# nunofonseca/fastq_utils

Hardware: AMD Instinct MI355X
Metric: Mreads/s validated (fastq_info, 150bp) (higher is better)
Workload: dtype u8

## Files before the change

### fastq_utils_amd/csrc/fqg_abi.hip

```cpp
#include <hip/hip_runtime.h>

#include <cstring>
#include <rocprim/rocprim.hpp>

#include <algorithm>
#include <cmath>
#include <memory>
#include <mutex>
#include <optional>
#include <cstdio>
#include <cstdlib>
#include <cstring>
#include <string>
#include <vector>

#include "fqg_device.h"
#include "fqg_kernels.hip"
#include "fqg_stream_kernels.hip"
#include "fqg_index_kernels.hip"
#include "fqg_names_build_kernels.hip"
#include "fqg_barcode_kernels.hip"
#include "fqg_census_kernels.hip"
#include "fqg_filter_kernels.hip"
#include "fqg_umi_kernels.hip"
// ... 710 lines not shown
  RecordDuties rd;
  int want_names;
  bool want_index;
  StreamOut so{};
  NameCapture nc{};
  ChunkRanks cr{};
  uint32_t n_parts = 1;
  int last_pct = 16;
  uint64_t early_line_cap = 0;
  uint64_t todo_steps_cap = 0;
  LinesArgs PA{};
  uint64_t n_newlines = 0, n_lines_all = 0, line_cap = 0, limit = 0;
  bool index_lost = false;

  uint32_t boot_span() const { return (uint32_t)std::min<uint64_t>(kStreamBootBytes, nbytes & ~255ull); }
  uint32_t part_begin(uint32_t part) const {
    if (part == 0 || n_parts <= 1) return part == 0 ? 0u : n_spans;
    if (part >= n_parts) return n_spans;
    const uint32_t last = std::min<uint32_t>(n_spans - (n_parts - 1), std::max<uint32_t>(1u, (uint32_t)((uint64_t)n_spans * (uint32_t)last_pct / 100u)));
    return (uint32_t)((uint64_t)(n_spans - last) * part / (n_parts - 1));
  }
  LinesArgs lines_args(const fqg_ctx* c, const ChunkRanks& cr, AccState* acc, unsigned long long* hist, const IndexMode& ix) const {
    LinesArgs A{};
    A.img = img;
    A.n = nbytes;
    A.cr = cr;
    A.stage = (const uint16_t*)c->stage.p;
    A.line_end = ix.line_end;
    A.line_cap = ix.line_cap;
    A.suspect_bits = sm.bits;
    A.suspect_cap = sm.cap;
    A.flags = sm.flags;
    A.space = rd.space;
    A.weight = rd.weight;
    A.acc = acc;
    A.hist = hist;
    A.no_index = ix.no_index ? 1u : 0u;
    A.index_only = 0u;
    A.keep_from = ix.keep_from;
    return A;
  }
};

ChunkRanks chunk_ranks(const fqg_ctx* c, uint32_t n_chunks) {
  ChunkRanks cr;
  cr.counts = (const uint32_t*)c->tile_counts.p;
  cr.local = (const uint32_t*)c->tile_local.p;
  cr.span_excl = (const unsigned long long*)c->span_sums.p;
  cr.n_chunks = n_chunks;
  return cr;
}

void fold_parted(fqg_ctx* c, AccState* dst, unsigned long long* dst_hist) {
  hipLaunchKernelGGL(k_acc_merge, dim3(64), dim3(kBlock), 0, c->stream, c->pipe_acc, c->pipe_hist, dst, dst_hist, dst ? 0 : 1);
  hipLaunchKernelGGL(k_acc_scratch_reset, dim3(1), dim3(1), 0, c->stream, c->pipe_acc);
  c->pipe_dirty = false;
}

int resident_per_cu(int& asked, const void* kernel) {
  if (!asked) {
    int nb = 0;
    if (hipOccupancyMaxActiveBlocksPerMultiprocessor(&nb, kernel, kBlock, 0) != hipSuccess || nb < 1) nb = 4;
    asked = nb;
  }
  return asked;
}

int stream_begin(fqg_ctx* c, StreamCall& s) {
  int rc;
  if ((rc = ensure(c, c->tile_counts, (size_t)s.n_chunks * 4))) return rc;
  if ((rc = ensure(c, c->tile_local, (size_t)s.n_chunks * 4))) return rc;
  if ((rc = ensure(c, c->span_sums, (size_t)s.n_spans * 8))) return rc;
  if ((rc = ensure(c, c->cinfo, (size_t)s.n_chunks * 4))) return rc;
  if ((rc = ensure(c, c->redo, (size_t)s.n_chunks * 4))) return rc;
  if ((rc = ensure(c, c->stage, (size_t)s.n_chunks * kStageCap * 2))) return rc;
  if ((rc = ensure(c, c->queue, (size_t)kStreamQueueCap * 8))) return rc;
  init_call_state(c);
  HIP_TRY(c, hipMemcpyAsync(c->d_cs, c->h_cs, sizeof(CallState), hipMemcpyHostToDevice, c->stream));
  s.so.counts = (uint32_t*)c->tile_counts.p;
  s.so.cinfo = (uint32_t*)c->cinfo.p;
  s.so.stage = (uint16_t*)c->stage.p;
  s.so.queue = (unsigned long long*)c->queue.p;
  s.so.queue_cap = kStreamQueueCap;
  s.cr = chunk_ranks(c, s.n_chunks);
  ProfScope ps(c, "k_stream_boot");
  hipLaunchKernelGGL(k_stream_boot, dim3(1), dim3(kBootBlock), 0, c->stream, s.img, s.boot_span(), c->d_cs);
  return 0;
}

int stream_name_setup(fqg_ctx* c, StreamCall& s) {
  int rc;
  if ((rc = read_call_state(c))) return rc;
  const double per_chunk = (double)(c->h_cs->boot_lines / 4 + 1) * (double)kChunkBytes / (double)std::max<uint32_t>(s.boot_span(), 1);
  uint32_t shift = 3;
  while (shift < 7 && (double)(1u << shift) < 1.25 * per_chunk + 1.0) ++shift;
  s.nc.K = 1u << shift;
  s.nc.fmt = s.rd.fmt;
  s.nc.is_pe = s.rd.is_pe;
  if ((rc = ensure(c, c->name_recs, ((size_t)s.n_chunks << shift) * (s.want_names == 2 ? kDigestWords : kNameRecWords) * 8))) return rc;
  if ((rc = ensure(c, c->name_hcount, (size_t)s.n_chunks * 2))) return rc;
  s.nc.recs = (unsigned long long*)c->name_recs.p;
  s.nc.hcount = (uint16_t*)c->name_hcount.p;
  c->names.k_shift = shift;
  return 0;
}

int stream_plan_parts(fqg_ctx* c, StreamCall& s) {
  int rc;
// ... 1764 lines not shown
```

### fastq_utils_amd/csrc/fqg_device.h

```cpp
#pragma once
#include <hip/hip_runtime.h>
#include <stdint.h>

#include "../../include/fqg.h"

namespace fqg {

constexpr int kWave = 64;
constexpr int kBlock = 256;
constexpr int kChunkBytes = 4096;
constexpr int kSlices = kChunkBytes / (kWave * 16);
constexpr int kScanSpan = 4096;
constexpr uint64_t kNoRecord = ~0ull;

constexpr uint32_t kFlagNul = 1u;
constexpr uint32_t kFlagCr = 2u;
constexpr uint32_t kFlagHigh = 8u;
constexpr uint32_t kFlagSuspectOverflow = 16u;
constexpr uint32_t kFlagStageOverflow = 32u;
constexpr uint32_t kFlagQueueOverflow = 64u;

constexpr int kStageCap = 256;
constexpr uint32_t kClsAt = 1u, kClsPlus = 2u;
constexpr uint32_t kInfoUnknown = 4u, kInfoRange = 8u, kInfoOneLine = 16u, kInfoNotBases = 32u;
// ... 2 lines not shown
  return (info & kInfoUnknown) || (info & 3u) != (rank0 & 3u);
}
__host__ __device__ inline bool chunk_info_range(uint32_t info, uint32_t rank0) {
  if (!(info & kInfoRange)) return false;
  return (info & kInfoOneLine) ? (rank0 & 3u) == 3u : true;
}

constexpr uint32_t kNameRecWords = 8;
constexpr uint32_t kNameRecText = 60;
constexpr uint32_t kNameInline = 56;
constexpr uint32_t kNoCapture = 0xFFFFu;
struct NameCapture {
  unsigned long long* recs;
  uint16_t* hcount;
  uint32_t K;
  int fmt, is_pe;
};
constexpr uint32_t kDigestWords = 2;
constexpr uint32_t kDigestText = 64;
constexpr uint32_t kDigestAt = 1u << 29, kDigestOk = 1u << 30;

__host__ __device__ constexpr uint64_t name_mul(uint32_t k) {
  return (0x9E3779B97F4A7C15ull + (uint64_t)k * 0xD1B54A32D192ED03ull) | 1ull;
}
__host__ __device__ constexpr uint32_t name_key_a(uint32_t k) { return (uint32_t)name_mul(k); }
__host__ __device__ constexpr uint32_t name_key_b(uint32_t k) { return (uint32_t)(name_mul(k) >> 32); }
__device__ __forceinline__ uint64_t name_word(uint64_t sum, uint64_t w, uint32_t k) {
  return sum + (uint64_t)((uint32_t)w + name_key_a(k)) * (uint64_t)((uint32_t)(w >> 32) + name_key_b(k));
}
__device__ __forceinline__ uint64_t name_seed(uint32_t n) { return 0x2545F4914F6CDD1Dull + (uint64_t)n; }
__device__ __forceinline__ uint64_t name_fin(uint64_t h) {
  const uint32_t hi = (uint32_t)(h >> 32), t = (uint32_t)h ^ hi;
  const uint64_t p = (uint64_t)t * 0xD6E8FEB9u, q = (uint64_t)hi * 0x85EBCA6Bu;
  return p ^ ((q << 32) | (q >> 32));
}

struct CallState {
  unsigned long long first_key;
  unsigned long long stop_record;
  unsigned long long n_newlines;
  unsigned long long aux0, aux1;
  unsigned long long list_count;
  unsigned int flags;
  unsigned int last_byte_is_nl;
  unsigned int qmin_byte, qmax_byte;
  unsigned long long queue_count;
  unsigned int redo_count;
  unsigned int boot_qmin, boot_qmax;
  unsigned int boot_lines;
  unsigned int pad_;
  unsigned long long trunc_record;
  unsigned long long part_newlines[4];
  unsigned long long lines_done_steps;
};

struct AccState {
  unsigned long long num_rds;
  unsigned long long min_rl;
  unsigned long long max_rl;
  unsigned int min_qbyte;
  unsigned int max_qbyte;
};

struct SuspectMap {
  uint32_t* bits;
  unsigned long long cap;
  unsigned int* flags;
};

struct FrameView {
  const uint8_t* img;
  uint64_t nbytes;
  const uint64_t* line_end;
  uint64_t n_lines;
  uint64_t n_records;
  uint32_t reframed = 0;
};

}
```

### fastq_utils_amd/csrc/fqg_stream_kernels.hip

```cpp
#include "fqg_device.h"

namespace fqg {

constexpr uint32_t kH = 0x80808080u;

__device__ __forceinline__ uint32_t pack_marks16(uint32_t m0, uint32_t m1, uint32_t m2, uint32_t m3) {
  uint32_t lo = __builtin_amdgcn_udot4(m0, 0x08040201u, 0u, false);
  lo = __builtin_amdgcn_udot4(m1, 0x80402010u, lo, false);
  uint32_t hi = __builtin_amdgcn_udot4(m2, 0x08040201u, 0u, false);
  hi = __builtin_amdgcn_udot4(m3, 0x80402010u, hi, false);
  return (lo >> 7) | (hi << 1);
}

__device__ __forceinline__ uint32_t nl_marks7(uint32_t w, uint32_t& bad) {
  const uint32_t x = w ^ 0x0A0A0A0Au;
  const uint32_t t = kH - x;
  const uint32_t c = t + 0x1F1F1F1Fu;
  bad = __builtin_amdgcn_bitop3_b32(bad, c, t, 0xF4);
  return t & kH;
}
__device__ __forceinline__ uint32_t or3(uint32_t a, uint32_t b, uint32_t c) { return __builtin_amdgcn_bitop3_b32(a, b, c, 0xFE); }

__device__ __forceinline__ uint32_t in_vgpr(uint32_t x) {
  uint32_t v;
  asm volatile("v_mov_b32 %0, %1" : "=v"(v) : "s"(x));
  return v;
}

__device__ __forceinline__ uint32_t not_acgtn7(uint32_t w) {
  const uint32_t want = __builtin_amdgcn_perm(0x474E7F54u, 0x437F417Fu, w & 0x07070707u);
  return ((w ^ want) + 0x7F7F7F7Fu) & kH;
}

__device__ __forceinline__ uint32_t in_range7(uint32_t w, uint32_t lob, uint32_t hihb, uint32_t kh = kH) {
  return ((w | kH) - lob) & (hihb - w) & kh;
}
__device__ __forceinline__ uint32_t in_range7a(uint32_t w, uint32_t lo_add, uint32_t hihb, uint32_t kh) {
  return (w + lo_add) & (hihb - w) & kh;
}

constexpr uint32_t kBootMax = 64u << 10;
constexpr int kBootBlock = 1024;
__global__ __launch_bounds__(kBootBlock) void k_stream_boot(const uint8_t* __restrict__ img, uint32_t span,
                                                            CallState* __restrict__ cs) {
  constexpr int kBootWaves = kBootBlock / kWave;
  __shared__ uint32_t s_cnt[kBootWaves];
  __shared__ __attribute__((aligned(16))) uint8_t s_img[kBootMax];
  const int lane = lane_id(), wv = threadIdx.x >> 6;
  const uint32_t part = span / kBootWaves;
  for (uint32_t o = threadIdx.x * 16u; o < span; o += kBootBlock * 16u)
    *reinterpret_cast<uint4*>(s_img + o) = *reinterpret_cast<const uint4*>(img + o);
  __syncthreads();
  const uint8_t* p = s_img + (uint64_t)wv * part;
// ... 2 lines not shown
  cnt = wave_sum(cnt);
  if (lane == 0) s_cnt[wv] = cnt;
  __syncthreads();
  uint32_t before = 0, total = 0;
  for (int w = 0; w < kBootWaves; ++w) {
    if (w < wv) before += s_cnt[w];
    total += s_cnt[w];
  }
  const uint32_t limit = total & ~3u;
  if (threadIdx.x == 0) cs->boot_lines = total;
  uint32_t line = before, qmin = 255, qmax = 0;
  for (uint32_t o = 0; o < part; o += kWave) {
    const uint32_t c = o + lane < part ? (uint32_t)p[o + lane] : 0u;
    const uint64_t bal = __ballot(o + lane < part && c == '\n');
    const uint32_t mine = line + (uint32_t)__builtin_popcountll(bal & ((1ull << lane) - 1ull));
    if ((mine & 3u) == 3u && mine < limit && c != '\n' && o + lane < part) {
      qmin = c < qmin ? c : qmin;
      qmax = c > qmax ? c : qmax;
    }
    line += (uint32_t)__builtin_popcountll(bal);
  }
#pragma unroll
  for (int d = 32; d > 0; d >>= 1) {
    const uint32_t a = __shfl_xor(qmin, d, 64), b = __shfl_xor(qmax, d, 64);
    qmin = a < qmin ? a : qmin;
    qmax = b > qmax ? b : qmax;
  }
  if (lane == 0 && qmin <= qmax) {
    atomicMin(&cs->boot_qmin, qmin);
    atomicMax(&cs->boot_qmax, qmax);
    atomicMin(&cs->qmin_byte, qmin);
    atomicMax(&cs->qmax_byte, qmax);
  }
}

struct StreamOut {
  uint32_t* counts;
  uint32_t* cinfo;
  uint16_t* stage;
  unsigned long long* queue;
  unsigned long long queue_cap;
};

__device__ __forceinline__ void queue_suspect(const StreamOut& o, CallState* cs, uint64_t pos) {
  if (__hip_atomic_load(&cs->queue_count, __ATOMIC_RELAXED, __HIP_MEMORY_SCOPE_AGENT) > o.queue_cap) return;
  const unsigned long long at = atomicAdd(&cs->queue_count, 1ull);
  if (at < o.queue_cap) o.queue[at] = pos;
}

constexpr int kHalves = 2;
constexpr int kLaneBytes = 32;
constexpr int kHalfBytes = kWave * kLaneBytes;

__device__ __forceinline__ uint32_t prefix_xor32(uint32_t x) {
  x ^= x << 1;
  x ^= x << 2;
  x ^= x << 4;
  x ^= x << 8;
  x ^= x << 16;
  return x;
}

__device__ __forceinline__ void type_masks32(uint32_t nl, uint32_t t0, uint32_t& M1, uint32_t& M3) {
  const uint32_t e = nl << 1;
  const uint32_t P = prefix_xor32(e);
  const uint32_t Q = prefix_xor32(e & ~P);
  const uint32_t a0 = 0u - (t0 & 1u), a1 = 0u - ((t0 >> 1) & 1u);
  const uint32_t L = P ^ a0;
  const uint32_t Hh = Q ^ a1 ^ (P & a0);
  M1 = ~Hh & L;
  M3 = Hh & L;
}

struct Piece32 {
  uint4 a, b;
};

constexpr uint32_t kCopyFront = 16, kCopyBack = 64;
constexpr uint32_t kCopyRow = kCopyFront + kChunkBytes + kCopyBack;

__device__ __forceinline__ uint32_t stage_entry(uint32_t ent, uint32_t c1) {
  return ent | ((c1 == '@' ? kClsAt : (c1 == '+' ? kClsPlus : 0u)) << 12);
}

template <uint32_t ABL>
__device__ __forceinline__ void stage_chunk(const uint8_t* __restrict__ img, uint64_t n, uint64_t cb, uint32_t chunk,
                                            const uint32_t (&nl)[kHalves], const uint32_t (&nl2)[kHalves],
                                            const uint32_t (&ex)[kHalves], uint32_t tot,
                                            uint16_t* __restrict__ slots, const uint8_t* __restrict__ copy,
                                            uint32_t tail, uint16_t* __restrict__ stage, bool interior) {
  const int lane = lane_id();
#pragma unroll
  for (int k = 0; k < kHalves; ++k) {
    uint32_t m = nl[k], r = ex[k];
    const uint32_t at = (uint32_t)k * kHalfBytes + (uint32_t)lane * kLaneBytes;
    while (m) {
      const uint32_t j = (uint32_t)__builtin_ctz(m);
      m &= m - 1;
      if (r < (uint32_t)kStageCap) slots[r] = (uint16_t)((at + j) | (((nl2[k] >> j) & 1u) << 14));
      ++r;
    }
  }
  __builtin_amdgcn_wave_barrier();
  uint16_t* dst = stage + (uint64_t)chunk * kStageCap;
  for (uint32_t i = lane; i < tot; i += kWave) {
    const uint32_t ent = slots[i];
    const uint32_t o = (ent & 0xFFFu) + 1;
    uint32_t c1 = 0;
    if (!(ABL & 4u)) {
      if (interior) c1 = o < (uint32_t)kChunkBytes ? (uint32_t)copy[o] : (tail & 0xFFu);
      else c1 = cb + o < n ? (uint32_t)img[cb + o] : 0u;
    }
    dst[i] = (uint16_t)stage_entry(ent, c1);
  }
}

template <int NAMES>
struct Pass1Lds {
  uint16_t slots[kBlock / kWave][kStageCap];
// ... 90 lines not shown
  ex[0] = (s01 & 0xFFFFu) - (c01 & 0xFFFFu);
  ex[1] = (t01 & 0xFFFFu) + (s01 >> 16) - (c01 >> 16);
  if (total > (uint32_t)kStageCap) flags |= kFlagStageOverflow;

  uint32_t tail_nl = 0;
  if (interior) {
    tail_nl = ((tail & 0xFFu) == '\n' ? 1u : 0u) | (((tail >> 8) & 0xFFu) == '\n' ? 2u : 0u);
  } else {
    for (uint64_t i = 0; i < 2; ++i)
      if (cb + kChunkBytes + i < n && img[cb + kChunkBytes + i] == '\n') tail_nl |= 1u << i;
  }
  uint32_t nl2[kHalves], cand[kHalves];
#pragma unroll
  for (int k = 0; k < kHalves; ++k) {
    uint32_t nxt = dpp0<0x130, 0xf, 0xf>(nl[k]);
    const uint32_t first_next = (uint32_t)__builtin_amdgcn_readlane(nl[k + 1 < kHalves ? k + 1 : k], 0);
    if (lane == 63) nxt = k + 1 < kHalves ? first_next : tail_nl;
    const uint32_t n1 = __builtin_amdgcn_alignbit(nxt, nl[k], 1);
    nl2[k] = __builtin_amdgcn_alignbit(nxt, nl[k], 2);
    cand[k] = nl[k] & nl2[k] & ~n1;
  }

  const uint32_t tot = total < (uint32_t)kStageCap ? total : (uint32_t)kStageCap;

  uint32_t info = kInfoUnknown;
  bool found = false;
  uint32_t t0 = 0;
  if (!(ABL & 1u) && interior && !(flags & kFlagHigh)) {
#pragma unroll
    for (int k = 0; k < kHalves; ++k) {
      const uint64_t bal = __ballot(cand[k] != 0);
      if (!found && bal) {
        const int l = __builtin_ctzll(bal);
        const uint32_t cl = (uint32_t)__builtin_amdgcn_readlane(cand[k], l);
        const uint32_t nll = (uint32_t)__builtin_amdgcn_readlane(nl[k], l);
        const uint32_t exl = (uint32_t)__builtin_amdgcn_readlane(ex[k], l);
        const uint32_t j = (uint32_t)__builtin_ctz(cl);
        const uint32_t a = exl + __popc(nll & ((1u << j) - 1u));
        t0 = (1u - a) & 3u;
        found = true;
      }
    }
    if (found) {
      info = t0;
      uint32_t lo = boot_lo, hi = boot_hi;
      if (lo > hi || lo > 127u) {
        lo = 127u;
        hi = 0u;
      }
      const uint32_t hihb_s = ((hi & 0x7Fu) | 0x80u) * 0x01010101u;
      const uint32_t lo_add = in_vgpr((0x80u - lo) * 0x01010101u), hihb = in_vgpr(hihb_s), khv = in_vgpr(kH);
      QRange q{0x00FF00FFu, 0x00FF00FFu, 0u, 0u};
      bool any_viol = false;
#pragma unroll
      for (int k = 0; k < kHalves; ++k) {
        uint32_t M1, M3;
        type_masks32(nl[k], t0 + ex[k], M1, M3);
        const uint4 &a = v[k].a, &b = v[k].b;
        const uint32_t inv = pack_marks16(not_acgtn7(a.x), not_acgtn7(a.y), not_acgtn7(a.z), not_acgtn7(a.w)) |
                             (pack_marks16(not_acgtn7(b.x), not_acgtn7(b.y), not_acgtn7(b.z), not_acgtn7(b.w)) << 16);
        const uint32_t bad = (ABL & 8u) ? 0u : inv & M1 & ~nl[k];
        if (bad) queue_suspect(o, cs, wb + (uint64_t)k * kHalfBytes + (uint32_t)__builtin_ctz(bad));
        const uint32_t okq =
            pack_marks16(in_range7a(a.x, lo_add, hihb, khv), in_range7a(a.y, lo_add, hihb, khv), in_range7a(a.z, lo_add, hihb, khv),
                         in_range7a(a.w, lo_add, hihb, khv)) |
            (pack_marks16(in_range7a(b.x, lo_add, hihb, khv), in_range7a(b.y, lo_add, hihb, khv), in_range7a(b.z, lo_add, hihb, khv),
                          in_range7a(b.w, lo_add, hihb, khv)) << 16);
        const uint32_t qm = (ABL & 16u) ? 0u : M3 & ~nl[k];
        if (__ballot((qm & ~okq) != 0)) {
          any_viol = true;
          qrange_accum(a, qm & 0xFFFFu, q);
          qrange_accum(b, qm >> 16, q);
        }
      }
      if (any_viol) {
        uint32_t qmin = pk_min_u16(q.mn_e, q.mn_o), qmax = pk_max_u16(q.mx_e, q.mx_o);
        qmin = (qmin & 0xFFFFu) < (qmin >> 16) ? (qmin & 0xFFFFu) : (qmin >> 16);
        qmax = (qmax & 0xFFFFu) > (qmax >> 16) ? (qmax & 0xFFFFu) : (qmax >> 16);
#pragma unroll
        for (int d = 32; d > 0; d >>= 1) {
          const uint32_t x = __shfl_xor(qmin, d, 64), y = __shfl_xor(qmax, d, 64);
          qmin = x < qmin ? x : qmin;
          qmax = y > qmax ? y : qmax;
        }
        if (qmin <= qmax) info |= kInfoRange | ((qmin & 0xFFu) << 8) | ((qmax & 0xFFu) << 16);
      }
    } else if (total == 0) {
      info = kInfoOneLine;
      uint32_t lo = boot_lo, hi = boot_hi;
      if (lo > hi || lo > 127u) {
        lo = 127u;
        hi = 0u;
      }
      const uint32_t lob = lo * 0x01010101u, hihb = ((hi & 0x7Fu) | 0x80u) * 0x01010101u;
      uint32_t not_base = 0, outside = 0;
#pragma unroll
      for (int k = 0; k < kHalves; ++k) {
        const uint32_t w[8] = {v[k].a.x, v[k].a.y, v[k].a.z, v[k].a.w, v[k].b.x, v[k].b.y, v[k].b.z, v[k].b.w};
#pragma unroll
        for (int j = 0; j < 8; ++j) {
          not_base |= not_acgtn7(w[j]);
          outside |= ~in_range7(w[j], lob, hihb) & kH;
        }
      }
      if (__ballot(not_base != 0)) info |= kInfoNotBases;
      if (__ballot(outside != 0)) {
        QRange q{0x00FF00FFu, 0x00FF00FFu, 0u, 0u};
#pragma unroll
        for (int k = 0; k < kHalves; ++k) {
          qrange_accum(v[k].a, 0xFFFFu, q);
          qrange_accum(v[k].b, 0xFFFFu, q);
        }
        uint32_t qmin = pk_min_u16(q.mn_e, q.mn_o), qmax = pk_max_u16(q.mx_e, q.mx_o);
        qmin = (qmin & 0xFFFFu) < (qmin >> 16) ? (qmin & 0xFFFFu) : (qmin >> 16);
        qmax = (qmax & 0xFFFFu) > (qmax >> 16) ? (qmax & 0xFFFFu) : (qmax >> 16);
#pragma unroll
        for (int d = 32; d > 0; d >>= 1) {
          const uint32_t x = __shfl_xor(qmin, d, 64), y = __shfl_xor(qmax, d, 64);
          qmin = x < qmin ? x : qmin;
          qmax = y > qmax ? y : qmax;
        }
// ... 280 lines not shown
  uint64_t n_newlines;
  uint64_t n_lines;
  uint64_t limit;
  uint32_t* suspect_bits;
  uint64_t suspect_cap;
  unsigned int* flags;
  int space;
  uint32_t weight;
  AccState* acc;
  unsigned long long* hist;
  int ablate;
  uint32_t no_index, index_only;
  uint64_t keep_from;
  uint64_t step_lo = 0, step_hi = 0;
};

constexpr int kLinesHist = 3072;
constexpr int kLinesPer = 2;
template <bool TODO>
__global__ __launch_bounds__(kBlock) void k_stream_lines(LinesArgs A, const uint8_t* __restrict__ todo) {
  __shared__ uint32_t s_hist[kLinesHist];
  __shared__ unsigned long long s_red[3][kBlock / kWave];
  __shared__ uint64_t s_wr0[kBlock / kWave][kWave];
  __shared__ uint32_t s_wcnt[kBlock / kWave][kWave];
  for (int i = threadIdx.x; i < kLinesHist; i += kBlock) s_hist[i] = 0;
  __syncthreads();
  const int lane = lane_id(), wv = (int)(threadIdx.x >> 6);
  uint32_t win0 = 0;
  const uint64_t n_groups = (A.n_lines + 4 * kWave - 1) / (4 * kWave);
  const uint64_t n_steps = (n_groups + kLinesPer - 1) / kLinesPer;
  const uint64_t wave0 = (uint64_t)blockIdx.x * (kBlock / kWave) + (threadIdx.x >> 6);
  const uint64_t n_waves = (uint64_t)gridDim.x * (kBlock / kWave);
  const double chunks_per_line = A.n_newlines ? (double)A.cr.n_chunks / (double)A.n_newlines : 0.0;
  unsigned long long n_ok = 0, min_rl = ~0ull, max_rl = 0;
  unsigned long long nx_se = 0;
  uint32_t nx_loc = 0, nx_cnt = 0, nx_win = 0;
  bool nx_in = false;
  auto window_request = [&](uint64_t step) {
    const uint64_t g = (step < n_steps ? step : n_steps - 1) * kLinesPer;
    const uint64_t Rw = g ? 4 * g * kWave - 1 : 0;
    const double est = (double)Rw * chunks_per_line;
    uint32_t cw = est > 2.0 ? (uint32_t)(est - 2.0) : 0u;
    if (cw + kWave > A.cr.n_chunks) cw = A.cr.n_chunks > (uint32_t)kWave ? A.cr.n_chunks - kWave : 0u;
    const uint32_t cm = cw + (uint32_t)lane;
    nx_in = cm < A.cr.n_chunks;
    const uint32_t cl = nx_in ? cm : A.cr.n_chunks - 1;
    nx_se = A.cr.span_excl[cl / kScanSpan];
    nx_loc = A.cr.local[cl];
    nx_cnt = A.cr.counts[cl];
    nx_win = cw;
  };
  if (!TODO && wave0 < n_steps) window_request(wave0);
  uint64_t blk = wave0 * (uint64_t)kWave, blk_cur = 0;
  unsigned long long marks = 0;
  for (uint64_t step = wave0;; step += n_waves) {
    if constexpr (TODO) {
      while (!marks && blk < n_steps) {
        const uint64_t s = blk + (uint64_t)lane;
        marks = __ballot(s < n_steps && todo[s] != 0);
        blk_cur = blk;
        blk += n_waves * (uint64_t)kWave;
      }
      if (!marks) break;
      step = blk_cur + (uint64_t)__builtin_ctzll(marks);
      marks &= marks - 1;
      window_request(step);
    } else if (step >= n_steps) break;
    uint64_t e[kLinesPer][5];
    uint32_t ent[kLinesPer][5];
    bool have[kLinesPer][5];
    s_wr0[wv][lane] = nx_in ? nx_se + nx_loc : ~0ull;
    s_wcnt[wv][lane] = nx_in ? nx_cnt : 0u;
    win0 = nx_win;
    __builtin_amdgcn_fence(__ATOMIC_RELEASE, "wavefront");
    __builtin_amdgcn_wave_barrier();
    uint64_t at[kLinesPer][5];
    bool ld[kLinesPer][5];
#pragma unroll
    for (int q = 0; q < kLinesPer; ++q) {
      const uint64_t g = step * kLinesPer + q;
      const uint64_t r = g * kWave + (uint64_t)lane;
      const uint64_t L0 = 4 * r;
      uint64_t R = r ? L0 - 1 : 0;
      const int k0 = r ? 0 : 1;
      e[q][0] = ~0ull;
      ent[q][0] = (kClsAt << 12);
      have[q][0] = r == 0;
      at[q][0] = 0;
      ld[q][0] = false;
      uint32_t c = 0, i = 0, cnt = 0;
      bool windowed = false;
      if (R < A.n_newlines) {
        if (R >= s_wr0[wv][0] && (R < s_wr0[wv][kWave - 1] + s_wcnt[wv][kWave - 1])) {
          uint32_t lo = 0, hi = kWave;
          while (hi - lo > 1) {
            const uint32_t mid = (lo + hi) >> 1;
            if (s_wr0[wv][mid] <= R) lo = mid;
            else hi = mid;
          }
          c = lo;
          i = (uint32_t)(R - s_wr0[wv][lo]);
          cnt = s_wcnt[wv][lo];
          windowed = true;
        } else {
          c = chunk_of_rank(A.cr, R, (uint32_t)((double)R * chunks_per_line));
          i = (uint32_t)(R - A.cr.rank0(c));
          cnt = A.cr.counts[c];
        }
      }
#pragma unroll
      for (int k = 0; k < 5; ++k) {
        if (k < k0) continue;
        at[q][k] = 0;
        ld[q][k] = false;
        if (R < A.n_newlines) {
          while (i >= cnt) {
            ++c;
// ... 13 lines not shown
          have[q][k] = true;
          ++i;
        } else if (R == A.n_newlines && A.n_lines > A.n_newlines) {
          ent[q][k] = 0;
          e[q][k] = A.n;
          have[q][k] = true;
        } else {
          ent[q][k] = 0;
          e[q][k] = 0;
          have[q][k] = false;
        }
        ++R;
      }
    }
    if constexpr (!TODO) window_request(step + n_waves);
    uint16_t raw[kLinesPer][5];
#pragma unroll
    for (int q = 0; q < kLinesPer; ++q)
#pragma unroll
      for (int k = 0; k < 5; ++k) raw[q][k] = A.stage[at[q][k]];
#pragma unroll
      for (int q = 0; q < kLinesPer; ++q)
#pragma unroll
        for (int k = 0; k < 5; ++k)
          if (ld[q][k]) ent[q][k] = raw[q][k];

    __builtin_amdgcn_wave_barrier();
#pragma unroll
    for (int q = 0; q < kLinesPer; ++q) {
      const uint64_t g = step * kLinesPer + q;
      const uint64_t r = g * kWave + (uint64_t)lane;
      const uint64_t L0 = 4 * r;
      {
        uint64_t R = r ? L0 - 1 : 0;
#pragma unroll
        for (int k = 0; k < 5; ++k) {
          if (k < (r ? 0 : 1)) continue;
          if (R < A.n_newlines) e[q][k] += (ent[q][k] & 0xFFFu);
          ++R;
        }
      }
      if ((A.ablate & 1) || (A.no_index && L0 + 4 <= A.keep_from)) {
      } else if (have[q][4] && L0 + 3 < A.line_cap) {
        typedef unsigned long long u64x2 __attribute__((ext_vector_type(2)));
        u64x2 lo2, hi2;
        lo2.x = e[q][1]; lo2.y = e[q][2]; hi2.x = e[q][3]; hi2.y = e[q][4];
        __builtin_nontemporal_store(lo2, reinterpret_cast<u64x2*>(A.line_end + L0));
        __builtin_nontemporal_store(hi2, reinterpret_cast<u64x2*>(A.line_end + L0 + 2));
      } else {
#pragma unroll
        for (int k = 1; k < 5; ++k)
          if (have[q][k] && L0 + k - 1 < A.line_cap) A.line_end[L0 + k - 1] = e[q][k];
      }
      bool sus = false, complete = have[q][4] && L0 + 3 < A.limit && !A.index_only, counted = false;
      uint64_t rl = 0;
      if (complete) {
        if (r == 0) sus |= A.img[0] != '@' || (A.n > 1 && A.img[1] == '\n');
        else sus |= !(((ent[q][0] >> 12) & 3u) == kClsAt && !((ent[q][0] >> 14) & 1u));
        sus |= !(((ent[q][2] >> 12) & 3u) == kClsPlus && ((ent[q][2] >> 14) & 1u));
        const uint64_t l0 = e[q][1] - e[q][0] - 1, l1 = e[q][2] - e[q][1] - 1, l2 = e[q][3] - e[q][2] - 1, l3 = e[q][4] - e[q][3] - 1;
        const uint32_t has_nl = e[q][4] < A.n ? 1u : 0u;
        sus |= l1 < 1 || l1 != l3 || A.space != FQG_SPACE_SEQ;
        sus |= l0 + 1 > FQG_MAX_LABEL_LENGTH - 1 || l2 + 1 > FQG_MAX_LABEL_LENGTH - 1 ||
               l1 + 1 > FQG_MAX_READ_LENGTH - 1 || l3 + has_nl > FQG_MAX_READ_LENGTH - 1;
        counted = A.acc && l1 + 1 <= FQG_MAX_READ_LENGTH - 1;
        if (counted) {
          rl = l1 + 1;
          ++n_ok;
          min_rl = rl < min_rl ? rl : min_rl;
          max_rl = rl > max_rl ? rl : max_rl;
        }
      }
      {
        const unsigned long long cm = __ballot(counted);
        if (cm) {
          const int first = __builtin_ctzll(cm);
          const uint32_t rl0 = (uint32_t)__builtin_amdgcn_readlane((uint32_t)rl, first);
          const bool with_first = counted && rl == (uint64_t)rl0;
          const unsigned long long same = __ballot(with_first);
          if (lane == first) {
            if (rl < (uint64_t)kLinesHist) atomicAdd(&s_hist[rl], (uint32_t)__builtin_popcountll(same));
            else atomicAdd(&A.hist[rl], (unsigned long long)A.weight * (unsigned long long)__builtin_popcountll(same));
          }
          if (counted && !with_first) {
            if (rl < (uint64_t)kLinesHist) atomicAdd(&s_hist[rl], 1u);
            else atomicAdd(&A.hist[rl], (unsigned long long)A.weight);
          }
        }
      }
      const unsigned long long sm = __ballot(sus);
      if (lane == 0 && sm) {
        const uint64_t w = g * 2;
        if ((g + 1) * kWave <= A.suspect_cap) {
          if ((uint32_t)sm) A.suspect_bits[w] = (uint32_t)sm;
          if ((uint32_t)(sm >> 32)) A.suspect_bits[w + 1] = (uint32_t)(sm >> 32);
        } else atomicOr(A.flags, kFlagSuspectOverflow);
      }
    }
  }
  if (!A.acc) return;
#pragma unroll
  for (int d = 32; d > 0; d >>= 1) {
    n_ok += __shfl_down(n_ok, d, 64);
    const unsigned long long a = __shfl_down(min_rl, d, 64), b = __shfl_down(max_rl, d, 64);
    min_rl = a < min_rl ? a : min_rl;
    max_rl = b > max_rl ? b : max_rl;
  }
// ... 36 lines not shown
};
__device__ __forceinline__ void stream_lines_fast_body(const LinesArgs& A, uint8_t* __restrict__ todo, uint32_t worker,
                                                       uint32_t n_workers, LinesFastLds& lds) {
  auto& s_hist = lds.hist;
  auto& s_red = lds.red;
  auto& s_ent = lds.ent;
  for (int i = threadIdx.x; i < kLinesHist; i += kBlock) s_hist[i] = 0;
  __syncthreads();
  const int lane = lane_id(), wv = (int)(threadIdx.x >> 6);
  const uint64_t n_groups = (A.n_lines + 4 * kWave - 1) / (4 * kWave);
  const uint64_t n_steps_all = (n_groups + kLinesPer - 1) / kLinesPer;
  const uint64_t n_steps = A.step_hi && A.step_hi < n_steps_all ? A.step_hi : n_steps_all;
  const uint64_t wave0 = A.step_lo + (uint64_t)worker * (kBlock / kWave) + (threadIdx.x >> 6);
  const uint64_t n_waves = (uint64_t)n_workers * (kBlock / kWave);
  const double chunks_per_line = A.n_newlines ? (double)A.cr.n_chunks / (double)A.n_newlines : 0.0;
  uint32_t n_ok32 = 0, min_rl32 = ~0u, max_rl32 = 0;
  unsigned long long nx_se = 0;
  uint32_t nx_loc = 0, nx_cnt = 0, nx_win = 0;
  bool nx_in = false;
  auto window_request = [&](uint64_t step) {
    const uint64_t g = (step < n_steps ? step : n_steps - 1) * kLinesPer;
    const uint64_t Rw = g ? 4 * g * kWave - 1 : 0;
    const double est = (double)Rw * chunks_per_line;
    uint32_t cw = est > 2.0 ? (uint32_t)(est - 2.0) : 0u;
    if (cw + kWave > A.cr.n_chunks) cw = A.cr.n_chunks > (uint32_t)kWave ? A.cr.n_chunks - kWave : 0u;
    const uint32_t cm = cw + (uint32_t)lane;
    nx_in = cm < A.cr.n_chunks;
    const uint32_t cl = nx_in ? cm : A.cr.n_chunks - 1;
    nx_se = A.cr.span_excl[cl / kScanSpan];
    nx_loc = A.cr.local[cl];
    nx_cnt = A.cr.counts[cl];
    nx_win = cw;
  };
  if (wave0 < n_steps) window_request(wave0);
  for (uint64_t step = wave0; step < n_steps; step += n_waves) {
    const uint64_t w0 = nx_in ? nx_se + nx_loc : ~0ull;
    const uint32_t wc = nx_in ? nx_cnt : 0u;
    const uint32_t win0 = (uint32_t)__builtin_amdgcn_readfirstlane((int)nx_win);
    const uint64_t rb = step * (uint64_t)(kWave * kLinesPer);
    const uint64_t Rlo = 4 * rb - 1, Rhi = 4 * rb + 4 * kWave * kLinesPer;
    bool fast = rb > 0 && Rhi <= A.n_newlines && Rhi <= A.limit && Rhi <= A.line_cap &&
                (rb / kWave + kLinesPer) * kWave <= A.suspect_cap;
    const unsigned long long b_lo = __ballot(w0 <= Rlo), b_hi = __ballot(w0 < Rhi);
    const int jfirst = __builtin_amdgcn_readfirstlane(__builtin_popcountll(b_lo) - 1);
    const int jlast = __builtin_amdgcn_readfirstlane(__builtin_popcountll(b_hi) - 1);
    const uint32_t n_cov = (uint32_t)(jlast - jfirst + 1);
    if (fast && b_lo != 0) {
      const unsigned long long many = __ballot(lane >= jfirst && lane <= jlast && wc > (uint32_t)kWave);
      const uint64_t last_r0 = readlane64(w0, jlast);
      const uint32_t last_cnt = (uint32_t)__builtin_amdgcn_readlane((int)wc, jlast);
      fast = many == 0 && n_cov <= (uint32_t)kFastSlots && last_r0 + last_cnt >= Rhi;
    } else fast = false;
    if (!__builtin_amdgcn_readfirstlane((int)fast)) {
      if (lane == 0) todo[step] = 1;
      window_request(step + n_waves);
      continue;
    }
    window_request(step + n_waves);
    const uint32_t rel0 = (uint32_t)(w0 - Rlo);
    constexpr uint32_t kDump = (uint32_t)kFastRanks;
    const uint16_t* const base0 = A.stage + (uint64_t)(win0 + (uint32_t)jfirst) * kStageCap;
    uint16_t raw[kFastSlots];
#pragma unroll
    for (int sl = 0; sl < kFastSlots; ++sl) {
      const uint32_t cj = (uint32_t)sl < n_cov ? (uint32_t)sl : 0u;
      const uint32_t cnt = (uint32_t)__builtin_amdgcn_readlane((int)wc, jfirst + (int)cj);
      raw[sl] = base0[cj * (uint32_t)kStageCap + ((uint32_t)lane < cnt ? (uint32_t)lane : 0u)];
    }
#pragma unroll
    for (int sl = 0; sl < kFastSlots; ++sl) {
      const uint32_t cj = (uint32_t)sl < n_cov ? (uint32_t)sl : 0u;
      const uint32_t cnt = (uint32_t)sl < n_cov ? (uint32_t)__builtin_amdgcn_readlane((int)wc, jfirst + (int)cj) : 0u;
      const uint32_t idx = (uint32_t)__builtin_amdgcn_readlane((int)rel0, jfirst + (int)cj) + (uint32_t)lane;
      s_ent[wv][((uint32_t)lane < cnt && idx < (uint32_t)kFastRanks) ? idx : kDump] = ((uint32_t)(jfirst + (int)cj) << 16) | (uint32_t)raw[sl];
    }
    __builtin_amdgcn_fence(__ATOMIC_RELEASE, "wavefront");
    __builtin_amdgcn_wave_barrier();
#pragma unroll
    for (int q = 0; q < kLinesPer; ++q) {
      const uint64_t g = step * kLinesPer + q;
      const uint64_t r = g * kWave + (uint64_t)lane;
      const uint64_t L0 = 4 * r;
      const uint32_t at = 4u * ((uint32_t)q * kWave + (uint32_t)lane);
      const uint4 e03 = *reinterpret_cast<const uint4*>(&s_ent[wv][at]);
      const uint32_t en[5] = {e03.x, e03.y, e03.z, e03.w, s_ent[wv][at + 4]};
      uint32_t rel[5];
#pragma unroll
      for (int k = 0; k < 5; ++k) rel[k] = ((en[k] >> 16) << 12) | (en[k] & 0xFFFu);
      if (!(A.ablate & 1) && !(A.no_index && L0 + 4 <= A.keep_from)) {
        typedef unsigned long long u64x2 __attribute__((ext_vector_type(2)));
        const uint64_t wbase = (uint64_t)win0 * kChunkBytes;
        u64x2 lo2, hi2;
        lo2.x = wbase + rel[1]; lo2.y = wbase + rel[2]; hi2.x = wbase + rel[3]; hi2.y = wbase + rel[4];
        __builtin_nontemporal_store(lo2, reinterpret_cast<u64x2*>(A.line_end + L0));
        __builtin_nontemporal_store(hi2, reinterpret_cast<u64x2*>(A.line_end + L0 + 2));
      }
      if (A.index_only) continue;
      bool sus = !(((en[0] >> 12) & 3u) == kClsAt && !((en[0] >> 14) & 1u));
      sus |= !(((en[2] >> 12) & 3u) == kClsPlus && ((en[2] >> 14) & 1u));
      const uint32_t l0 = rel[1] - rel[0] - 1, l1 = rel[2] - rel[1] - 1, l2 = rel[3] - rel[2] - 1, l3 = rel[4] - rel[3] - 1;
      sus |= l1 < 1 || l1 != l3 || A.space != FQG_SPACE_SEQ;
      sus |= l0 + 1 > FQG_MAX_LABEL_LENGTH - 1 || l2 + 1 > FQG_MAX_LABEL_LENGTH - 1 ||
             l1 + 1 > FQG_MAX_READ_LENGTH - 1 || l3 + 1 > FQG_MAX_READ_LENGTH - 1;
      const bool counted = A.acc && l1 + 1 <= FQG_MAX_READ_LENGTH - 1;
      const uint32_t rl = l1 + 1;
      if (counted) {
        ++n_ok32;
// ... 27 lines not shown
    __builtin_amdgcn_wave_barrier();
  }
  if (!A.acc) return;
  unsigned long long n_ok = n_ok32, min_rl = min_rl32 == ~0u ? ~0ull : (unsigned long long)min_rl32, max_rl = max_rl32;
#pragma unroll
  for (int d = 32; d > 0; d >>= 1) {
    n_ok += __shfl_down(n_ok, d, 64);
    const unsigned long long a = __shfl_down(min_rl, d, 64), b = __shfl_down(max_rl, d, 64);
    min_rl = a < min_rl ? a : min_rl;
    max_rl = b > max_rl ? b : max_rl;
  }
  if (lane == 0) {
    s_red[0][threadIdx.x >> 6] = n_ok;
    s_red[1][threadIdx.x >> 6] = min_rl;
    s_red[2][threadIdx.x >> 6] = max_rl;
  }
  __syncthreads();
  if (threadIdx.x == 0) {
    for (int w = 1; w < kBlock / kWave; ++w) {
      n_ok += s_red[0][w];
      min_rl = s_red[1][w] < min_rl ? s_red[1][w] : min_rl;
      max_rl = s_red[2][w] > max_rl ? s_red[2][w] : max_rl;
    }
    if (n_ok) {
      atomicAdd(&A.acc->num_rds, n_ok * A.weight);
      if (min_rl < A.acc->min_rl) atomicMin(&A.acc->min_rl, min_rl);
      if (max_rl > A.acc->max_rl) atomicMax(&A.acc->max_rl, max_rl);
    }
  }
  for (int i = threadIdx.x; i < kLinesHist; i += kBlock) {
    const uint32_t cc = s_hist[i];
    if (cc) atomicAdd(&A.hist[i], (unsigned long long)cc * A.weight);
  }
}

__global__ __launch_bounds__(kBlock) __attribute__((amdgpu_waves_per_eu(7, 8))) void k_stream_lines_fast(LinesArgs A, uint8_t* __restrict__ todo) {
  __shared__ LinesFastLds lds;
  stream_lines_fast_body(A, todo, blockIdx.x, gridDim.x, lds);
}

template <int NAMES>
__global__ __launch_bounds__(kBlock) __attribute__((amdgpu_waves_per_eu(7, 8))) void k_stream_pass1_lines(
    const uint8_t* __restrict__ img, uint64_t n, uint32_t chunk_first, uint32_t n_chunks, StreamOut o, CallState* __restrict__ cs,
    LinesArgs A, uint8_t* __restrict__ todo, uint32_t line_workers, uint32_t part , NameCapture nc) {
  union Lds {
    Pass1Lds<NAMES> p1;
    LinesFastLds lf;
  };
  __shared__ Lds lds;
  if (blockIdx.x >= line_workers) {
    stream_pass1_body<0u, NAMES>(img, n, n_chunks, o, cs, nc, chunk_first / (kBlock / kWave) + (blockIdx.x - line_workers), lds.p1);
    return;
  }
  if (__hip_atomic_load(&cs->flags, __ATOMIC_RELAXED, __HIP_MEMORY_SCOPE_AGENT) & (kFlagNul | kFlagCr | kFlagHigh | kFlagStageOverflow)) return;
  const unsigned long long R = cs->part_newlines[part], R0 = part ? cs->part_newlines[part - 1] : 0ull;
  const double per_chunk = (double)R / (double)(chunk_first ? chunk_first : 1u);
  if (per_chunk > 60.0 || per_chunk < 32.0) return;
  A.n_newlines = R;
  A.n_lines = R;
  A.limit = R & ~3ull;
  A.cr.n_chunks = chunk_first;
  A.step_lo = R0 / (uint64_t)(4 * kWave * kLinesPer);
  A.step_hi = R / (uint64_t)(4 * kWave * kLinesPer);
  if (blockIdx.x == 0 && threadIdx.x == 0) cs->lines_done_steps = A.step_hi;
  if (A.step_hi <= A.step_lo) return;
  stream_lines_fast_body(A, todo, blockIdx.x, line_workers, lds.lf);
}

__global__ __launch_bounds__(kBlock) void k_acc_merge(AccState* __restrict__ src, unsigned long long* __restrict__ src_hist,
                                                      AccState* __restrict__ dst, unsigned long long* __restrict__ dst_hist,
                                                      int discard) {
  __shared__ unsigned long long s_lo, s_hi;
  if (threadIdx.x == 0) {
    s_lo = src->min_rl;
    s_hi = src->max_rl;
  }
  __syncthreads();
  const unsigned long long lo = s_lo, hi = s_hi;
  if (lo <= hi)
    for (unsigned long long i = lo + (unsigned long long)blockIdx.x * kBlock + threadIdx.x; i <= hi; i += (unsigned long long)gridDim.x * kBlock) {
      const unsigned long long v = src_hist[i];
      if (v) {
        if (!discard && dst_hist) atomicAdd(&dst_hist[i], v);
        src_hist[i] = 0;
      }
    }
  if (!discard && dst && blockIdx.x == 0 && threadIdx.x == 0 && src->num_rds) {
    atomicAdd(&dst->num_rds, src->num_rds);
    atomicMin(&dst->min_rl, src->min_rl);
    atomicMax(&dst->max_rl, src->max_rl);
  }
}
__global__ void k_acc_scratch_reset(AccState* __restrict__ a) {
  a->num_rds = 0;
  a->min_rl = FQG_MAX_READ_LENGTH;
  a->max_rl = 0;
  a->min_qbyte = 255;
  a->max_qbyte = 0;
}

__global__ __launch_bounds__(kBlock) void k_suspect_list(const uint32_t* __restrict__ bits, uint64_t n_records,
                                                         unsigned long long* __restrict__ list,
                                                         unsigned long long list_cap,
                                                         unsigned long long* __restrict__ list_count,
                                                         AccState* __restrict__ acc, const CallState* __restrict__ cs) {
  const uint64_t n_words = (n_records + 31) / 32;
  const uint64_t stride = (uint64_t)gridDim.x * kBlock;
  const int lane = lane_id();
  for (uint64_t w0 = (uint64_t)blockIdx.x * kBlock + (threadIdx.x & ~63u); w0 < n_words; w0 += stride) {
    const uint64_t w = w0 + (uint64_t)lane;
    uint32_t m = w < n_words ? bits[w] : 0u;
    if (w * 32 + 32 > n_records) m &= w * 32 < n_records ? (uint32_t)((1ull << (n_records - w * 32)) - 1ull) : 0u;
    const uint32_t cnt = (uint32_t)__popc(m);
    uint32_t incl = cnt;
#pragma unroll
    for (int d = 1; d < 64; d <<= 1) {
      const uint32_t o = __shfl_up(incl, d, 64);
      if (lane >= d) incl += o;
    }
    const uint32_t total = (uint32_t)__builtin_amdgcn_readlane((int)incl, 63);
    if (!total) continue;
    unsigned long long base = 0;
    if (lane == 0) base = atomicAdd(list_count, (unsigned long long)total);
    base = ((unsigned long long)(uint32_t)__builtin_amdgcn_readfirstlane((int)(uint32_t)(base >> 32)) << 32) |
           (uint32_t)__builtin_amdgcn_readfirstlane((int)(uint32_t)base);
    unsigned long long at = base + (incl - cnt);
    while (m) {
      const uint32_t j = (uint32_t)__builtin_ctz(m);
      m &= m - 1;
      if (at < list_cap) list[at] = w * 32 + j;
      ++at;
    }
  }
  if (acc && blockIdx.x == 0 && threadIdx.x == 0 && cs->qmin_byte <= cs->qmax_byte) {
    atomicMin(&acc->min_qbyte, cs->qmin_byte);
    atomicMax(&acc->max_qbyte, cs->qmax_byte);
  }
}

__global__ __launch_bounds__(kBlock) void k_stream_queue(const unsigned long long* __restrict__ queue,
                                                         unsigned long long queue_cap,
                                                         const uint64_t* __restrict__ line_end, uint64_t n_lines,
                                                         uint64_t n_records, SuspectMap suspect,
// ... 22 lines not shown
```

Baseline: 12380.

## Add two-newline fast path for type masks, fuse acc merge/reset, chain part steps

Adds a cheaper arithmetic way to compute line-type parities when a 32-byte lane holds at most two newlines, selected wave-uniformly via a ballot, with the prefix-xor path kept as fallback. Folds the accumulator scratch reset into a single-block merge kernel, removing one launch per fold. Tracks per-part completed line steps so later parts run the lines-fast worker only when earlier parts finished contiguously. Marks steps that failed only in index-only mode with a distinct todo value so they are not double-counted. The single-block merge may be slower on wide length histograms, and the new part bookkeeping adds state that must stay consistent.

```diff
diff --git a/fastq_utils_amd/csrc/fqg_abi.hip b/fastq_utils_amd/csrc/fqg_abi.hip
--- a/fastq_utils_amd/csrc/fqg_abi.hip
+++ b/fastq_utils_amd/csrc/fqg_abi.hip
@@ -786,8 +786,7 @@
 }
 
 void fold_parted(fqg_ctx* c, AccState* dst, unsigned long long* dst_hist) {
-  hipLaunchKernelGGL(k_acc_merge, dim3(64), dim3(kBlock), 0, c->stream, c->pipe_acc, c->pipe_hist, dst, dst_hist, dst ? 0 : 1);
-  hipLaunchKernelGGL(k_acc_scratch_reset, dim3(1), dim3(1), 0, c->stream, c->pipe_acc);
+  hipLaunchKernelGGL(k_acc_merge, dim3(1), dim3(kMergeBlock), 0, c->stream, c->pipe_acc, c->pipe_hist, dst, dst_hist, dst ? 0 : 1);
   c->pipe_dirty = false;
 }
 
diff --git a/fastq_utils_amd/csrc/fqg_device.h b/fastq_utils_amd/csrc/fqg_device.h
--- a/fastq_utils_amd/csrc/fqg_device.h
+++ b/fastq_utils_amd/csrc/fqg_device.h
@@ -78,6 +78,7 @@
   unsigned long long trunc_record;
   unsigned long long part_newlines[4];
   unsigned long long lines_done_steps;
+  unsigned long long part_done_steps[4];
 };
 
 struct AccState {
diff --git a/fastq_utils_amd/csrc/fqg_stream_kernels.hip b/fastq_utils_amd/csrc/fqg_stream_kernels.hip
--- a/fastq_utils_amd/csrc/fqg_stream_kernels.hip
+++ b/fastq_utils_amd/csrc/fqg_stream_kernels.hip
@@ -1,4 +1,5 @@
 #include "fqg_device.h"
+#include "fqg_type_masks.h"
 
 namespace fqg {
 
@@ -107,19 +108,12 @@
 constexpr int kLaneBytes = 32;
 constexpr int kHalfBytes = kWave * kLaneBytes;
 
-__device__ __forceinline__ uint32_t prefix_xor32(uint32_t x) {
-  x ^= x << 1;
-  x ^= x << 2;
-  x ^= x << 4;
-  x ^= x << 8;
-  x ^= x << 16;
-  return x;
-}
-
+template <bool TWO>
 __device__ __forceinline__ void type_masks32(uint32_t nl, uint32_t t0, uint32_t& M1, uint32_t& M3) {
-  const uint32_t e = nl << 1;
-  const uint32_t P = prefix_xor32(e);
-  const uint32_t Q = prefix_xor32(e & ~P);
+  const uint32_t e = nl + nl;
+  uint32_t P, Q;
+  if (TWO) type_parities_two(e, P, Q);
+  else type_parities_shift(e, P, Q);
   const uint32_t a0 = 0u - (t0 & 1u), a1 = 0u - ((t0 >> 1) & 1u);
   const uint32_t L = P ^ a0;
   const uint32_t Hh = Q ^ a1 ^ (P & a0);
@@ -316,21 +310,28 @@
       const uint32_t lo_add = in_vgpr((0x80u - lo) * 0x01010101u), hihb = in_vgpr(hihb_s), khv = in_vgpr(kH);
       QRange q{0x00FF00FFu, 0x00FF00FFu, 0u, 0u};
       bool any_viol = false;
+      const bool two = !(ABL & 32u) && __ballot(((c01 + 0x7FFD7FFDu) & 0x80008000u) != 0) == 0;
+      uint32_t M1[kHalves], M3[kHalves];
+      if (two) {
+#pragma unroll
+        for (int k = 0; k < kHalves; ++k) type_masks32<true>(nl[k], t0 + ex[k], M1[k], M3[k]);
+      } else {
+#pragma unroll
+        for (int k = 0; k < kHalves; ++k) type_masks32<false>(nl[k], t0 + ex[k], M1[k], M3[k]);
+      }
 #pragma unroll
       for (int k = 0; k < kHalves; ++k) {
-        uint32_t M1, M3;
-        type_masks32(nl[k], t0 + ex[k], M1, M3);
         const uint4 &a = v[k].a, &b = v[k].b;
         const uint32_t inv = pack_marks16(not_acgtn7(a.x), not_acgtn7(a.y), not_acgtn7(a.z), not_acgtn7(a.w)) |
                              (pack_marks16(not_acgtn7(b.x), not_acgtn7(b.y), not_acgtn7(b.z), not_acgtn7(b.w)) << 16);
-        const uint32_t bad = (ABL & 8u) ? 0u : inv & M1 & ~nl[k];
+        const uint32_t bad = (ABL & 8u) ? 0u : inv & M1[k] & ~nl[k];
         if (bad) queue_suspect(o, cs, wb + (uint64_t)k * kHalfBytes + (uint32_t)__builtin_ctz(bad));
         const uint32_t okq =
             pack_marks16(in_range7a(a.x, lo_add, hihb, khv), in_range7a(a.y, lo_add, hihb, khv), in_range7a(a.z, lo_add, hihb, khv),
                          in_range7a(a.w, lo_add, hihb, khv)) |
             (pack_marks16(in_range7a(b.x, lo_add, hihb, khv), in_range7a(b.y, lo_add, hihb, khv), in_range7a(b.z, lo_add, hihb, khv),
                           in_range7a(b.w, lo_add, hihb, khv)) << 16);
-        const uint32_t qm = (ABL & 16u) ? 0u : M3 & ~nl[k];
+        const uint32_t qm = (ABL & 16u) ? 0u : M3[k] & ~nl[k];
         if (__ballot((qm & ~okq) != 0)) {
           any_viol = true;
           qrange_accum(a, qm & 0xFFFFu, q);
@@ -717,17 +718,22 @@
   };
   if (!TODO && wave0 < n_steps) window_request(wave0);
   uint64_t blk = wave0 * (uint64_t)kWave, blk_cur = 0;
-  unsigned long long marks = 0;
+  unsigned long long marks = 0, marks_index = 0;
+  bool index_step = false;
   for (uint64_t step = wave0;; step += n_waves) {
     if constexpr (TODO) {
       while (!marks && blk < n_steps) {
         const uint64_t s = blk + (uint64_t)lane;
-        marks = __ballot(s < n_steps && todo[s] != 0);
+        const uint32_t mk = s < n_steps ? (uint32_t)todo[s] : 0u;
+        marks = __ballot(mk != 0);
+        marks_index = __ballot(mk == 2u);
         blk_cur = blk;
         blk += n_waves * (uint64_t)kWave;
       }
       if (!marks) break;
-      step = blk_cur + (uint64_t)__builtin_ctzll(marks);
+      const int mb = __builtin_ctzll(marks);
+      step = blk_cur + (uint64_t)mb;
+      index_step = ((marks_index >> mb) & 1ull) != 0;
       marks &= marks - 1;
       window_request(step);
     } else if (step >= n_steps) break;
@@ -847,7 +853,7 @@
         for (int k = 1; k < 5; ++k)
           if (have[q][k] && L0 + k - 1 < A.line_cap) A.line_end[L0 + k - 1] = e[q][k];
       }
-      bool sus = false, complete = have[q][4] && L0 + 3 < A.limit && !A.index_only, counted = false;
+      bool sus = false, complete = have[q][4] && L0 + 3 < A.limit && !A.index_only && !index_step, counted = false;
       uint64_t rl = 0;
       if (complete) {
         if (r == 0) sus |= A.img[0] != '@' || (A.n > 1 && A.img[1] == '\n');
@@ -990,7 +996,10 @@
       fast = many == 0 && n_cov <= (uint32_t)kFastSlots && last_r0 + last_cnt >= Rhi;
     } else fast = false;
     if (!__builtin_amdgcn_readfirstlane((int)fast)) {
-      if (lane == 0) todo[step] = 1;
+      if (lane == 0) {
+        if (!A.index_only) todo[step] = 1;
+        else if (!todo[step]) todo[step] = 2;
+      }
       window_request(step + n_waves);
       continue;
     }
@@ -1124,43 +1133,52 @@
     stream_pass1_body<0u, NAMES>(img, n, n_chunks, o, cs, nc, chunk_first / (kBlock / kWave) + (blockIdx.x - line_workers), lds.p1);
     return;
   }
-  if (__hip_atomic_load(&cs->flags, __ATOMIC_RELAXED, __HIP_MEMORY_SCOPE_AGENT) & (kFlagNul | kFlagCr | kFlagHigh | kFlagStageOverflow)) return;
+  const unsigned long long done = part ? cs->part_done_steps[part - 1] : 0ull;
   const unsigned long long R = cs->part_newlines[part], R0 = part ? cs->part_newlines[part - 1] : 0ull;
   const double per_chunk = (double)R / (double)(chunk_first ? chunk_first : 1u);
-  if (per_chunk > 60.0 || per_chunk < 32.0) return;
   A.n_newlines = R;
   A.n_lines = R;
   A.limit = R & ~3ull;
   A.cr.n_chunks = chunk_first;
   A.step_lo = R0 / (uint64_t)(4 * kWave * kLinesPer);
   A.step_hi = R / (uint64_t)(4 * kWave * kLinesPer);
-  if (blockIdx.x == 0 && threadIdx.x == 0) cs->lines_done_steps = A.step_hi;
-  if (A.step_hi <= A.step_lo) return;
+  const bool flagged =
+      (__hip_atomic_load(&cs->flags, __ATOMIC_RELAXED, __HIP_MEMORY_SCOPE_AGENT) & (kFlagNul | kFlagCr | kFlagHigh | kFlagStageOverflow)) != 0;
+  const bool runs = !flagged && per_chunk <= 60.0 && per_chunk >= 32.0 && done == A.step_lo;
+  if (blockIdx.x == 0 && threadIdx.x == 0) {
+    const unsigned long long upto = runs ? (unsigned long long)A.step_hi : done;
+    cs->part_done_steps[part < 4u ? part : 3u] = upto;
+    cs->lines_done_steps = upto;
+  }
+  if (!runs || A.step_hi <= A.step_lo) return;
   stream_lines_fast_body(A, todo, blockIdx.x, line_workers, lds.lf);
 }
 
-__global__ __launch_bounds__(kBlock) void k_acc_merge(AccState* __restrict__ src, unsigned long long* __restrict__ src_hist,
-                                                      AccState* __restrict__ dst, unsigned long long* __restrict__ dst_hist,
-                                                      int discard) {
-  __shared__ unsigned long long s_lo, s_hi;
-  if (threadIdx.x == 0) {
-    s_lo = src->min_rl;
-    s_hi = src->max_rl;
-  }
-  __syncthreads();
-  const unsigned long long lo = s_lo, hi = s_hi;
+constexpr int kMergeBlock = 1024;
+__global__ __launch_bounds__(kMergeBlock) void k_acc_merge(AccState* __restrict__ src, unsigned long long* __restrict__ src_hist,
+                                                           AccState* __restrict__ dst, unsigned long long* __restrict__ dst_hist,
+                                                           int discard) {
+  const unsigned long long lo = src->min_rl, hi = src->max_rl, num = src->num_rds;
   if (lo <= hi)
-    for (unsigned long long i = lo + (unsigned long long)blockIdx.x * kBlock + threadIdx.x; i <= hi; i += (unsigned long long)gridDim.x * kBlock) {
+    for (unsigned long long i = lo + threadIdx.x; i <= hi; i += kMergeBlock) {
       const unsigned long long v = src_hist[i];
       if (v) {
         if (!discard && dst_hist) atomicAdd(&dst_hist[i], v);
         src_hist[i] = 0;
       }
     }
-  if (!discard && dst && blockIdx.x == 0 && threadIdx.x == 0 && src->num_rds) {
-    atomicAdd(&dst->num_rds, src->num_rds);
-    atomicMin(&dst->min_rl, src->min_rl);
-    atomicMax(&dst->max_rl, src->max_rl);
+  __syncthreads();
+  if (threadIdx.x == 0) {
+    if (!discard && dst && num) {
+      atomicAdd(&dst->num_rds, num);
+      atomicMin(&dst->min_rl, lo);
+      atomicMax(&dst->max_rl, hi);
+    }
+    src->num_rds = 0;
+    src->min_rl = FQG_MAX_READ_LENGTH;
+    src->max_rl = 0;
+    src->min_qbyte = 255;
+    src->max_qbyte = 0;
   }
 }
 __global__ void k_acc_scratch_reset(AccState* __restrict__ a) {
diff --git a/fastq_utils_amd/csrc/fqg_type_masks.h b/fastq_utils_amd/csrc/fqg_type_masks.h
--- /dev/null
+++ b/fastq_utils_amd/csrc/fqg_type_masks.h
@@ -0,0 +1,33 @@
+#pragma once
+#include <stdint.h>
+
+#if defined(__HIPCC__) || defined(__CUDACC__)
+#define FQG_TM_FN __host__ __device__ __forceinline__
+#else
+#define FQG_TM_FN inline
+#endif
+
+namespace fqg {
+
+FQG_TM_FN uint32_t prefix_xor32(uint32_t x) {
+  x ^= x << 1;
+  x ^= x << 2;
+  x ^= x << 4;
+  x ^= x << 8;
+  x ^= x << 16;
+  return x;
+}
+
+FQG_TM_FN void type_parities_shift(uint32_t e, uint32_t& P, uint32_t& Q) {
+  P = prefix_xor32(e);
+  Q = prefix_xor32(e & ~P);
+}
+
+FQG_TM_FN void type_parities_two(uint32_t e, uint32_t& P, uint32_t& Q) {
+  const uint32_t low = e & (0u - e);
+  const uint32_t rest = e ^ low;
+  Q = 0u - rest;
+  P = (0u - low) ^ Q;
+}
+
+}
```

Result: faster. 12540 (median of 6 runs) (+1.3%).
